# Jumpat/SegAnyGAussians

Measured on AMD Instinct MI355X. Metric: train views/sec (fwd+bwd), 1080p, 1M Gaussians, 32-D features, higher is better.
Workload: dtype f32; 1 GPU; BASELINE cfg3: 1000000 Gaussians, 1920x1080, 32-D features, fwd+bwd, 1 view/GPU/step; parallelism=view-sharded x1

## Files before the change

### seganygaussians_amd/csrc/binning.h

```cpp
#pragma once

#include <type_traits>

#include "common.h"
#include "cull.h"

namespace mirast {

__device__ __forceinline__ uint32_t wave_inclusive_scan(uint32_t v, int lane)
{
#pragma unroll
    for (int o = 1; o < 64; o <<= 1) {
        const uint32_t t = __shfl_up(v, o, 64);
        if (lane >= o) v += t;
    }
    return v;
}

template <int CTRL, int ROW_MASK, int BANK_MASK>
__device__ __forceinline__ uint32_t dpp_or_zero(uint32_t v)
{
    return (uint32_t)__builtin_amdgcn_update_dpp(0, (int)v, CTRL, ROW_MASK, BANK_MASK, false);
}
template <bool MAX = false>
// ... 17 lines not shown

struct RectWork {
    uint32_t* prefix;
    uint32_t* rx;
    uint32_t* ry;
    uint32_t* wsum;
};

template <int NT = 1024, typename F>
__device__ __forceinline__ void for_each_tile_balanced(const RectWork& rw, int tid, uint2 rmin, uint2 rmax, uint32_t count, F&& f)
{
    const int lane = tid & 63, wave = tid >> 6;
    uint32_t incl = wave_inclusive_scan(count, lane);
    if (lane == 63) rw.wsum[wave] = incl;
    __syncthreads();
    uint32_t woff = 0, total = 0;
#pragma unroll
    for (int w = 0; w < NT / 64; w++) {
        const uint32_t c = rw.wsum[w];
        woff += w < wave ? c : 0u;
        total += c;
    }
    incl += woff;
    rw.prefix[tid] = incl;
    rw.rx[tid] = rmin.x | ((rmax.x - rmin.x) << 16);
    rw.ry[tid] = rmin.y;
    __syncthreads();
    for (uint32_t k = (uint32_t)tid; k < total; k += NT) {
        int lo = 0;
#pragma unroll
        for (int step = NT / 2; step >= 1; step >>= 1)
            if (rw.prefix[lo + step - 1] <= k) lo += step;
        const uint32_t packed = rw.rx[lo];
        const uint32_t w = packed >> 16, x0 = packed & 0xFFFFu, y0 = rw.ry[lo];
        const uint32_t prev = lo == 0 ? 0u : rw.prefix[lo - 1];
        const uint32_t i = k - prev;
        const uint32_t row = (uint32_t)(((float)i + 0.5f) * __builtin_amdgcn_rcpf((float)w));
        const uint32_t col = i - row * w;
        f((uint32_t)lo, x0 + col, y0 + row);
    }
    __syncthreads();
}

constexpr int ID_BITS = 28;
constexpr uint32_t ID_MASK = (1u << ID_BITS) - 1u;
constexpr int BIN_MAX_WG = 256;
constexpr int BIN_THREADS = 1024;
constexpr int BIN_LEAN_WG = 256;
constexpr int BIN_MAX_TILES = 22 * 1024 - 64;
constexpr int BIN_MAX_TILES_TOTAL = 40 * 1024 - 128;

__host__ __device__ inline bool band_geometry(uint32_t gx, uint32_t gy, uint32_t max_head_words, uint32_t& band_h, uint32_t& nbands)
{
    band_h = (gy + 15u) / 16u;
    if (band_h < 1u) band_h = 1u;
    while (band_h > 1u && (band_h + 1u) * (gx + 2u) > max_head_words) band_h--;
    nbands = (gy + band_h - 1u) / band_h;
    return nbands <= (uint32_t)MAX_BANDS && (band_h + 1u) * (gx + 2u) <= max_head_words;
}

__device__ __forceinline__ void band_plan(const int* __restrict__ r_slots, uint32_t nbands, uint32_t nwg, uint32_t* s_plan, int lane)
{
    uint32_t cnt = 0;
    if ((uint32_t)lane < nbands)
        for (int k = 0; k < R_SLOTS; k++) cnt += (uint32_t)r_slots[k * R_SLOT_STRIDE + R_SLOT_BANDS + lane];
    uint32_t total = cnt;
#pragma unroll
    for (int o = 32; o >= 1; o >>= 1) total += (uint32_t)__shfl_xor((int)total, o, 64);
    const uint32_t avail = nwg > nbands ? nwg - nbands : 0u;
    uint32_t n = (uint32_t)lane < nbands ? 1u + (total ? (uint32_t)(((uint64_t)cnt * avail) / total) : 0u) : 0u;
    if (nwg < nbands) n = (uint32_t)lane < nwg ? 1u : 0u;
    uint32_t incl = n;
#pragma unroll
    for (int o = 1; o < 64; o <<= 1) {
        const uint32_t t = (uint32_t)__shfl_up((int)incl, o, 64);
        if (lane >= o) incl += t;
    }
    if ((uint32_t)lane < nbands) s_plan[lane] = incl - n;
    if ((uint32_t)lane == nbands) s_plan[nbands] = incl;
}

constexpr int NR_TOTAL = 0, NR_LONGEST = 1, NR_VERIFY = 2, NR_KEY_BITS = 3, NR_RUN_BOUNDS = 4;

__global__ void __launch_bounds__(1024) tile_ranges_kernel(int ntiles_all, const uint32_t* __restrict__ tile_total,
                                                           uint2* __restrict__ ranges, int* __restrict__ num_rendered,
                                                           const int* __restrict__ r_slots, int* __restrict__ host_out = nullptr,
                                                           uint32_t* __restrict__ zero_a = nullptr, uint32_t* __restrict__ zero_b = nullptr,
                                                           uint32_t* __restrict__ run_bounds = nullptr ,
                                                           uint32_t run_cap = 0, uint32_t run_fix = 0)
{
    extern __shared__ uint32_t s_val[];
    __shared__ uint32_t s_wave[16];
    __shared__ uint32_t s_wave_w[16];
    __shared__ uint32_t s_bound[9];
    const bool weighted = run_bounds != nullptr && run_cap > 0u && ntiles_all <= BIN_MAX_TILES_TOTAL;
    __shared__ uint32_t s_maxcount;
    const int tid = threadIdx.x, lane = tid & 63, wave = tid >> 6;
    if (tid < 9) s_bound[tid] = xcd_run_start((uint32_t)tid, (uint32_t)ntiles_all);
    if (tid == 0) s_maxcount = 0;
    if (wave == 15 && r_slots != nullptr) {
        uint32_t inv_min = (uint32_t)r_slots[(lane % R_SLOTS) * R_SLOT_STRIDE + 1];
        uint32_t mx = (uint32_t)r_slots[(lane % R_SLOTS) * R_SLOT_STRIDE + 2];
#pragma unroll
        for (int o = 32; o >= 1; o >>= 1) {
            inv_min = max(inv_min, (uint32_t)__shfl_xor((int)inv_min, o, 64));
            mx = max(mx, (uint32_t)__shfl_xor((int)mx, o, 64));
        }
        const uint32_t kmin = ~inv_min;
        const uint32_t diff = mx >= kmin ? (mx ^ kmin) : 0u;
        if (lane == 0) num_rendered[NR_KEY_BITS] = diff ? 32 - __builtin_clz(diff) : 0;
    }
    uint32_t carry = 0;
    for (int seg0 = 0; seg0 < ntiles_all; seg0 += BIN_MAX_TILES_TOTAL) {
        const int ntiles = min(BIN_MAX_TILES_TOTAL, ntiles_all - seg0);
        for (int i = tid; i < ntiles; i += 1024) s_val[i] = tile_total[seg0 + i];
        __syncthreads();
        const int per = (ntiles + 1023) / 1024;
        const int i0 = min(ntiles, tid * per), i1 = min(ntiles, i0 + per);
        uint32_t sum = 0, mx = 0, wsum = 0;
        for (int i = i0; i < i1; i++) {
            const uint32_t c = s_val[i];
            s_val[i] = sum;
            sum += c;
            mx = max(mx, c);
            wsum += min(c, run_cap) + run_fix;
        }
        const uint32_t incl = wave_inclusive_scan(sum, lane);
        const uint32_t incl_w = weighted ? wave_inclusive_scan(wsum, lane) : 0u;
        if (lane == 63) {
            s_wave[wave] = incl;
            s_wave_w[wave] = incl_w;
        }
#pragma unroll
        for (int o = 32; o >= 1; o >>= 1) mx = max(mx, (uint32_t)__shfl_xor((int)mx, o, 64));
        __syncthreads();
        if (lane == 0 && mx) atomicMax(&s_maxcount, mx);
        uint32_t woff = 0, total = 0;
#pragma unroll
        for (int w = 0; w < 16; w++) {
            const uint32_t c = s_wave[w];
            woff += w < wave ? c : 0u;
            total += c;
        }
        const uint32_t piece_base = carry + woff + incl - sum;
        for (int i = i0; i < i1; i++) s_val[i] += piece_base;
        if (tid == 0) s_val[ntiles] = carry + total;
        uint32_t woff_w = 0, total_w = 0;
        if (weighted) {
#pragma unroll
            for (int w = 0; w < 16; w++) {
                const uint32_t c = s_wave_w[w];
                woff_w += w < wave ? c : 0u;
                total_w += c;
            }
        }
        __syncthreads();
        if (weighted && total_w > 0u) {
            const uint64_t w_lo = 8ull * (uint64_t)(woff_w + incl_w - wsum), w_hi = 8ull * (uint64_t)(woff_w + incl_w);
#pragma unroll
            for (uint32_t k = 1; k < 8u; k++) {
                const uint64_t want = (uint64_t)k * (uint64_t)total_w;
                if (w_lo < want && want <= w_hi) {
                    uint64_t wacc = w_lo;
                    int i = i0;
                    for (; i < i1; i++) {
                        wacc += 8ull * (uint64_t)(min(s_val[i + 1] - s_val[i], run_cap) + run_fix);
                        if (wacc >= want) break;
                    }
                    s_bound[k] = (uint32_t)min(i + 1, i1);
                }
            }
        }
        for (int i = tid; i < ntiles; i += 1024) {
            const uint32_t lo = s_val[i], hi = s_val[i + 1];
            ranges[seg0 + i] = hi > lo ? make_uint2(lo, hi) : make_uint2(0u, 0u);
            if (zero_a != nullptr) {
                zero_a[seg0 + i] = 0u;
                zero_b[seg0 + i] = 0u;
            }
        }
        carry += total;
        __syncthreads();
    }
    if (run_bounds != nullptr) {
        const uint32_t n = (uint32_t)ntiles_all;
        if (tid == 0) {
            uint32_t bb[9];
#pragma unroll
            for (int k = 1; k < 8; k++) bb[k] = s_bound[k];
            const uint32_t maxrun = xcd_max_run(n);
            bb[0] = 0u;
            bb[8] = n;
#pragma unroll
            for (uint32_t k = 1; k < 8u; k++) {
                const uint32_t prev = bb[k - 1], need = (8u - k) * maxrun;
                bb[k] = min(max(bb[k], max(prev, n > need ? n - need : 0u)), min(n, prev + maxrun));
            }
#pragma unroll
            for (int k = 0; k < 9; k++) {
                run_bounds[k] = bb[k];
                if (host_out != nullptr) host_out[NR_RUN_BOUNDS + k] = (int)bb[k];
            }
        }
    }
    if (tid == 0) {
        num_rendered[NR_TOTAL] = (int)carry;
        num_rendered[NR_LONGEST] = (int)s_maxcount;
        if (host_out != nullptr) {
            host_out[NR_TOTAL] = (int)carry;
            host_out[NR_LONGEST] = (int)s_maxcount;
        }
    }
}

constexpr int MI_FP_MAX = 8;
constexpr int FP_BLOCKS = 128;
struct FingerprintArgs {
    const uint32_t* ptr[MI_FP_MAX];
    unsigned long long words[MI_FP_MAX];
};
__global__ void __launch_bounds__(256) fingerprint_kernel(FingerprintArgs a, unsigned long long* __restrict__ out)
{
    const int k = blockIdx.y;
    const uint32_t* p = a.ptr[k];
    const unsigned long long n = a.words[k];
    unsigned long long sum = 0;
    for (unsigned long long i = (unsigned long long)blockIdx.x * 256ull + threadIdx.x; i < n; i += (unsigned long long)FP_BLOCKS * 256ull) {
        uint32_t x = p[i] ^ ((uint32_t)i * 0x9E3779B1u + (uint32_t)(i >> 32));
        x ^= x >> 16;
        x *= 0x85EBCA6Bu;
        x ^= x >> 13;
        x *= 0xC2B2AE35u;
        x ^= x >> 16;
        sum += (unsigned long long)x * 0x9E3779B97F4A7C15ull + i;
    }
    __shared__ unsigned long long s_part[4];
#pragma unroll
    for (int o = 32; o >= 1; o >>= 1) sum += __shfl_xor(sum, o, 64);
    if ((threadIdx.x & 63) == 0) s_part[threadIdx.x >> 6] = sum;
    __syncthreads();
    if (threadIdx.x == 0) out[k * FP_BLOCKS + blockIdx.x] = s_part[0] + s_part[1] + s_part[2] + s_part[3];
}

__global__ void __launch_bounds__(256) reuse_image_state_kernel(uint32_t ntiles, const uint2* __restrict__ src_ranges,
                                                                const int* __restrict__ src_words, uint2* __restrict__ ranges,
                                                                int* __restrict__ words, uint32_t* __restrict__ zero_a,
                                                                uint32_t* __restrict__ zero_b)
{
    const uint32_t t = blockIdx.x * 256u + threadIdx.x;
    if (t < ntiles) {
        ranges[t] = src_ranges[t];
        zero_a[t] = 0u;
        zero_b[t] = 0u;
    }
    if (t < 16u) words[t] = src_words[t];
}

struct __attribute__((aligned(16))) BlendRec {
    float2 xy;
    uint32_t id;
    uint32_t pm;
    float4 co;
};
static_assert(sizeof(BlendRec) == 32, "BlendRec must be 32 bytes");

__device__ __forceinline__ BlendRec list_record(const uint32_t* __restrict__ lst, const BlendRec* __restrict__ index_rec, int i)
{
    const uint32_t e = lst[i];
    BlendRec r = index_rec[e & ID_MASK];
    r.id = e & ID_MASK;
    r.pm = ((uint32_t)i << 4) | (e >> ID_BITS);
    return r;
}

inline int bin_workgroups(int P)
{
    const int blocks = (P + BIN_THREADS - 1) / BIN_THREADS;
    return blocks < 1 ? 1 : (blocks > BIN_MAX_WG ? BIN_MAX_WG : blocks);
}

template <bool NOCULL = false>
__global__ void __launch_bounds__(BIN_THREADS) bin_ranks_kernel(int P, const BlendRec* __restrict__ index_rec,
                                                                const uint32_t* __restrict__ depth_key,
                                                                const uint32_t* __restrict__ partial,
                                                                const uint2* __restrict__ ranges,
                                                                uint2* __restrict__ entries, uint32_t gx, uint32_t gy,
                                                                uint32_t by0, uint32_t by1)
{
    extern __shared__ uint32_t s_dyn[];
    const int ntiles = (int)(gx * (by1 - by0));
    const int tile0 = (int)(gx * by0);
    const int ntiles_all = (int)(gx * gy);
    uint32_t* s_cnt = s_dyn;
// ... 681 lines not shown
```

### seganygaussians_amd/csrc/geometry.h

```cpp
#pragma once

#include "binning.h"
#include "common.h"

namespace mirast {

__device__ constexpr float SH_C0 = 0.28209479177387814f;
__device__ constexpr float SH_C1 = 0.4886025119029199f;
__device__ constexpr float SH_C2[5] = {1.0925484305920792f, -1.0925484305920792f, 0.31539156525252005f,
                                       -1.0925484305920792f, 0.5462742152960396f};
__device__ constexpr float SH_C3[7] = {-0.5900435899266435f, 2.890611442640554f, -0.4570457994644658f,
                                       0.3731763325901154f, -0.4570457994644658f, 1.445305721320277f,
                                       -0.5900435899266435f};

__device__ __forceinline__ void computeCov3D(const float3 scale, float mod, const float4 rot, float* cov3D)
{
    Mat3 S = {{{1.0f, 0, 0}, {0, 1.0f, 0}, {0, 0, 1.0f}}};
    S.m[0][0] = mod * scale.x;
    S.m[1][1] = mod * scale.y;
    S.m[2][2] = mod * scale.z;
    float r = rot.x, x = rot.y, y = rot.z, z = rot.w;
    Mat3 R = {{{1.f - 2.f * (y * y + z * z), 2.f * (x * y - r * z), 2.f * (x * z + r * y)},
               {2.f * (x * y + r * z), 1.f - 2.f * (x * x + z * z), 2.f * (y * z - r * x)},
               {2.f * (x * z - r * y), 2.f * (y * z + r * x), 1.f - 2.f * (x * x + y * y)}}};
// ... 5 lines not shown
    cov3D[3] = Sigma.m[1][1];
    cov3D[4] = Sigma.m[1][2];
    cov3D[5] = Sigma.m[2][2];
}

struct Cov2DCtx {
    float3 t;
    float txtz, tytz;
    Mat3 T, Vrk, W, cov;
};

__device__ __forceinline__ void cov2d_common(const float3& mean, const ViewParams& vp, const float* cov3D, Cov2DCtx& c)
{
    float3 t = transformPoint4x3(mean, vp.view);
    const float limx = 1.3f * vp.tan_fovx;
    const float limy = 1.3f * vp.tan_fovy;
    c.txtz = t.x / t.z;
    c.tytz = t.y / t.z;
    t.x = fminf(limx, fmaxf(-limx, c.txtz)) * t.z;
    t.y = fminf(limy, fmaxf(-limy, c.tytz)) * t.z;
    Mat3 J = {{{vp.focal_x / t.z, 0.0f, -(vp.focal_x * t.x) / (t.z * t.z)},
               {0.0f, vp.focal_y / t.z, -(vp.focal_y * t.y) / (t.z * t.z)},
               {0, 0, 0}}};
    c.W = {{{vp.view[0], vp.view[4], vp.view[8]}, {vp.view[1], vp.view[5], vp.view[9]}, {vp.view[2], vp.view[6], vp.view[10]}}};
    c.T = m3mul(c.W, J);
    c.Vrk = {{{cov3D[0], cov3D[1], cov3D[2]}, {cov3D[1], cov3D[3], cov3D[4]}, {cov3D[2], cov3D[4], cov3D[5]}}};
    c.cov = m3mul(m3mul(m3transpose(c.T), m3transpose(c.Vrk)), c.T);
    c.cov.m[0][0] += 0.3f;
    c.cov.m[1][1] += 0.3f;
    c.t = t;
}

__device__ __forceinline__ float3 computeColorFromSH(int idx, int deg, const float3 pos, const ViewParams& vp,
                                                     const float* sh, uint8_t* clamped)
{
    float3 dir = make_float3(pos.x - vp.campos[0], pos.y - vp.campos[1], pos.z - vp.campos[2]);
    float len = sqrtf(dir.x * dir.x + dir.y * dir.y + dir.z * dir.z);
    dir.x = dir.x / len;
    dir.y = dir.y / len;
    dir.z = dir.z / len;
    const float x = dir.x, y = dir.y, z = dir.z;
    float res[3];
#pragma unroll
    for (int c = 0; c < 3; c++) {
#define SH(k) sh[(k) * 3 + c]
        float result = SH_C0 * SH(0);
        if (deg > 0) {
            result = result - SH_C1 * y * SH(1) + SH_C1 * z * SH(2) - SH_C1 * x * SH(3);
            if (deg > 1) {
                float xx = x * x, yy = y * y, zz = z * z;
                float xy = x * y, yz = y * z, xz = x * z;
                result = result + SH_C2[0] * xy * SH(4) + SH_C2[1] * yz * SH(5) + SH_C2[2] * (2.0f * zz - xx - yy) * SH(6) +
                         SH_C2[3] * xz * SH(7) + SH_C2[4] * (xx - yy) * SH(8);
                if (deg > 2) {
                    result = result + SH_C3[0] * y * (3.0f * xx - yy) * SH(9) + SH_C3[1] * xy * z * SH(10) +
                             SH_C3[2] * y * (4.0f * zz - xx - yy) * SH(11) +
                             SH_C3[3] * z * (2.0f * zz - 3.0f * xx - 3.0f * yy) * SH(12) +
                             SH_C3[4] * x * (4.0f * zz - xx - yy) * SH(13) + SH_C3[5] * z * (xx - yy) * SH(14) +
                             SH_C3[6] * x * (xx - 3.0f * yy) * SH(15);
                }
            }
        }
#undef SH
        result += 0.5f;
        clamped[3 * idx + c] = (result < 0);
        res[c] = fmaxf(result, 0.0f);
    }
    return make_float3(res[0], res[1], res[2]);
}

__global__ void __launch_bounds__(256) preprocess_fwd_kernel(
    int P, int D, int M, const float* __restrict__ orig_points, const float* __restrict__ scales,
    const float* __restrict__ rotations, const float* __restrict__ opacities, const float* __restrict__ shs,
    uint8_t* __restrict__ clamped, const float* __restrict__ cov3D_precomp, int colors_given, ViewParams vp,
    int* __restrict__ radii, float2* __restrict__ points_xy_image, float* __restrict__ depths,
    float* __restrict__ cov3Ds, float* __restrict__ rgb, float4* __restrict__ conic_opacity,
    uint32_t* __restrict__ tiles_touched, uint32_t* __restrict__ depth_key, BlendRec* __restrict__ index_rec,
    int* __restrict__ r_slots, int prefiltered, int* __restrict__ culled_prefiltered, unsigned long long* __restrict__ band_bits,
    uint32_t band_h, uint32_t nbands, uint32_t* __restrict__ tile_total, uint32_t ntiles)
{
    const int idx = blockIdx.x * blockDim.x + threadIdx.x;
    __shared__ uint32_t s_band[MAX_BANDS];
    if (threadIdx.x < MAX_BANDS) s_band[threadIdx.x] = 0u;
    if ((uint32_t)idx < ntiles) tile_total[idx] = 0u;
    extern __shared__ float s_sh[];
    const int sh_row = 3 * M + 4;
    if (!colors_given) {
        const int rows = min((int)blockDim.x, P - (int)(blockIdx.x * blockDim.x));
        const size_t base = (size_t)blockIdx.x * blockDim.x * 3 * M;
        const int nfl = rows * 3 * M;
        if ((3 * M) % 4 == 0 && (reinterpret_cast<uintptr_t>(shs) & 15) == 0) {
            for (int i = 4 * (int)threadIdx.x; i < nfl; i += 4 * (int)blockDim.x) {
                const float4 v = *reinterpret_cast<const float4*>(shs + base + i);
                *reinterpret_cast<float4*>(&s_sh[(i / (3 * M)) * sh_row + i % (3 * M)]) = v;
            }
        } else {
            for (int i = (int)threadIdx.x; i < nfl; i += (int)blockDim.x) s_sh[(i / (3 * M)) * sh_row + i % (3 * M)] = shs[base + i];
        }
        __syncthreads();
    }
    int my_radii = 0;
    uint32_t my_tiles = 0;
    uint32_t my_key = 0xFFFFFFFFu;
    uint2 rect_min = make_uint2(0, 0), rect_max = make_uint2(0, 0);
    if (idx < P) do {
        const float3 p_orig = make_float3(orig_points[3 * idx], orig_points[3 * idx + 1], orig_points[3 * idx + 2]);
        const float3 p_view = transformPoint4x3(p_orig, vp.view);
        if (p_view.z <= 0.2f) {
            if (prefiltered) atomicAdd(culled_prefiltered, 1);
            break;
        }
        const float4 p_hom = transformPoint4x4(p_orig, vp.proj);
        const float p_w = 1.0f / (p_hom.w + 0.0000001f);
        const float3 p_proj = make_float3(p_hom.x * p_w, p_hom.y * p_w, p_hom.z * p_w);

        float cov3D[6];
        if (cov3D_precomp != nullptr) {
#pragma unroll
            for (int i = 0; i < 6; i++) cov3D[i] = cov3D_precomp[(size_t)idx * 6 + i];
        } else {
            const float3 s = make_float3(scales[3 * idx], scales[3 * idx + 1], scales[3 * idx + 2]);
            const float4 q = reinterpret_cast<const float4*>(rotations)[idx];
            computeCov3D(s, vp.scale_modifier, q, cov3D);
#pragma unroll
            for (int i = 0; i < 6; i++) cov3Ds[(size_t)idx * 6 + i] = cov3D[i];
        }
        Cov2DCtx c;
        cov2d_common(p_orig, vp, cov3D, c);
        const float3 cov = make_float3(c.cov.m[0][0], c.cov.m[0][1], c.cov.m[1][1]);
        const float det = (cov.x * cov.z - cov.y * cov.y);
        if (det == 0.0f) break;
        const float det_inv = 1.f / det;
        const float3 conic = make_float3(cov.z * det_inv, -cov.y * det_inv, cov.x * det_inv);
        const float mid = 0.5f * (cov.x + cov.z);
        const float lambda1 = mid + sqrtf(fmaxf(0.1f, mid * mid - det));
        const float lambda2 = mid - sqrtf(fmaxf(0.1f, mid * mid - det));
        const float my_radius = ceilf(3.f * sqrtf(fmaxf(lambda1, lambda2)));
        const float2 point_image = make_float2(ndc2Pix(p_proj.x, vp.W), ndc2Pix(p_proj.y, vp.H));
        uint2 rmin, rmax;
        getRect(point_image.x, point_image.y, f2i(my_radius), rmin, rmax, vp.grid_x, vp.grid_y);
        if ((rmax.x - rmin.x) * (rmax.y - rmin.y) == 0) break;

        if (!colors_given) {
            const float3 col = computeColorFromSH(idx, D, p_orig, vp, s_sh + threadIdx.x * sh_row, clamped);
            rgb[idx * 3 + 0] = col.x;
            rgb[idx * 3 + 1] = col.y;
            rgb[idx * 3 + 2] = col.z;
        }
        depths[idx] = p_view.z;
        my_radii = f2i(my_radius);
        points_xy_image[idx] = point_image;
        conic_opacity[idx] = make_float4(conic.x, conic.y, conic.z, opacities[idx]);
        my_tiles = (rmax.y - rmin.y) * (rmax.x - rmin.x);
        if (my_radii > 0) {
            getRect(point_image.x, point_image.y, my_radii, rect_min, rect_max, vp.grid_x, vp.grid_y);
            my_key = __float_as_uint(p_view.z);
            BlendRec rec;
            rec.xy = point_image;
            rec.id = my_key;
            rec.pm = (uint32_t)my_radii;
            rec.co = make_float4(conic.x, conic.y, conic.z, opacities[idx]);
            index_rec[idx] = rec;
        }
    } while (0);
    uint32_t my_bands = 0u;
    if (my_radii > 0 && rect_max.y > rect_min.y && rect_max.x > rect_min.x) {
        const uint32_t b0 = rect_min.y / band_h, b1 = (rect_max.y - 1u) / band_h;
// ... 318 lines not shown
```

### seganygaussians_amd/csrc/mi_rast.hip

```cpp
#include "../../include/mi_rast.h"
#include "../../include/mi_knn_smooth.h"
#include "../../include/mi_knn.h"
#include "../../include/mi_contrastive.h"
#include "../../include/mi_mask_scales.h"
#include "../../include/mi_segment.h"
#include "../../include/mi_photometric.h"

#include <hip/hip_runtime.h>

#include <algorithm>
#include <atomic>
#include <cstdio>
#include <cstdlib>
#include <cstring>
#include <mutex>
#include <string>
#include <vector>

#include "binning.h"
#include "knn_smooth.h"
#include "knn.h"
#include "blend_bwd.h"
#include "blend_bwd_wave.h"
#include "blend_bwd_feat.h"
// ... 208 lines not shown
    mi_rast_image_layout(W, H, off);
    ImgPtrs m;
    m.final_T = (float*)(base + off[MI_IMG_FINAL_T]);
    m.n_contrib = (uint32_t*)(base + off[MI_IMG_N_CONTRIB]);
    m.ranges = (uint2*)(base + off[MI_IMG_RANGES]);
    m.tile_consumed = (uint32_t*)(base + off[MI_IMG_TILE_CONSUMED]);
    m.tile_count = (uint32_t*)(base + off[MI_IMG_TILE_COUNT]);
    m.tile_cursor = (uint32_t*)(base + off[MI_IMG_TILE_CURSOR]);
    m.num_rendered = (int*)(base + off[MI_IMG_NUM_RENDERED]);
    m.tile_nsurv = (uint32_t*)(base + off[MI_IMG_TILE_NSURV]);
    m.run_bounds = reinterpret_cast<uint32_t*>(m.num_rendered + R_SLOTS * R_SLOT_STRIDE + NR_RUN_BOUNDS);
    m.longest_run = 0;
    return m;
}
BinPtrs bin_from(char* base, int R)
{
    size_t off[MI_BIN_NFIELDS];
    mi_rast_binning_layout(R, off);
    BinPtrs b;
    b.entries = (uint2*)(base + off[MI_BIN_ENTRIES]);
    b.scratch = (uint2*)(base + off[MI_BIN_SCRATCH]);
    b.blend_list = (uint32_t*)(base + off[MI_BIN_BLEND_LIST]);
    return b;
}

std::atomic<bool> g_attr_set[MAX_DEVICES];
std::mutex g_attr_mutex;

constexpr int MAX_CHANNELS = 256;
constexpr int MAX_CHANNEL_BLOCKS = MAX_CHANNELS / 16;
inline size_t bwd_pack_bytes(int P)
{
    return (size_t)(P > 0 ? P : 1) * 8 * sizeof(float) + MAX_CHANNEL_BLOCKS * 8 * XCD_QUEUE_STRIDE * sizeof(uint32_t);
}
bool channels_supported(int c) { return c >= 1 && c <= MAX_CHANNELS; }
int channel_block(int rem) { return rem >= 64 ? 64 : (rem >= 32 ? 32 : 16); }

constexpr int RUN_MODEL_CAP = 768;
constexpr int RUN_MODEL_FIX = 128;
inline uint32_t longest_of(const int* bounds, uint32_t ntiles)
{
    uint32_t longest = 0;
    for (int x = 0; x < 8; x++) {
        const uint32_t a = (uint32_t)bounds[x], b = (uint32_t)bounds[x + 1];
        longest = std::max(longest, b >= a ? b - a : 0u);
    }
    return std::min(std::max(longest, (ntiles + 7u) >> 3), xcd_max_run(ntiles));
}

int geometry_and_binning(mi_rast_resize_fn geometry_buffer, void* geometry_user, mi_rast_resize_fn binning_buffer,
                         void* binning_user, mi_rast_resize_fn image_buffer, void* image_user, int P, int D, int M,
                         int W, int H, const float* means3D, const float* shs, int colors_given,
                         const float* opacities, const float* scales, const float* rotations,
                         const float* cov3D_precomp, const ViewParams& vp, int prefiltered, int* radii, int debug,
                         int flags, hipStream_t stream, GeomPtrs& geom, ImgPtrs& img, BinPtrs& bin, int* num_rendered)
{
    const int dev = current_device();
    if (dev < 0) return fail(MI_RAST_ERR_HIP, "hipGetDevice failed (or device ordinal >= 64)");
    HostSync& g_host_sync = g_host_sync_tl[dev];
    size_t goff[MI_GEOM_NFIELDS], ioff[MI_IMG_NFIELDS];
    const size_t geom_size = mi_rast_geometry_layout(P, goff);
    char* geom_base = geometry_buffer(geom_size, geometry_user);
    if (!geom_base) return fail(MI_RAST_ERR_ALLOC, "geometry buffer callback returned NULL");
    geom = geom_from(geom_base, P);
    const size_t img_size = mi_rast_image_layout(W, H, ioff);
    char* img_base = image_buffer(img_size, image_user);
    if (!img_base) return fail(MI_RAST_ERR_ALLOC, "image buffer callback returned NULL");
    img = img_from(img_base, W, H);

    int* cull_counter = geom.cull_counter;
    if (prefiltered) HIP_TRY(hipMemsetAsync(cull_counter, 0, sizeof(int), stream));
    const int ntiles = (int)(vp.grid_x * vp.grid_y);
    if (P >= (1 << ID_BITS)) return fail(MI_RAST_ERR_INVALID, "more than 2^28 Gaussians");
    if (vp.grid_x > 1023u || vp.grid_y > 2047u)
        return fail(MI_RAST_ERR_INVALID, "image too large: more than 1023 tiles across or 2047 tiles down");
    const uint32_t band_rows = std::min<uint32_t>(vp.grid_y, std::max<uint32_t>(1u, (uint32_t)BIN_MAX_TILES / (vp.grid_x + 2u) - 1u));
    const uint32_t nbands = (vp.grid_y + band_rows - 1) / band_rows;
    uint32_t lean_band_h = 1, lean_nbands = 1;
    if (!band_geometry(vp.grid_x, vp.grid_y, SPAN_MAX_HEAD_WORDS, lean_band_h, lean_nbands))
        return fail(MI_RAST_ERR_INVALID, "image too large for the banded binning passes (more than 24 bands of tile rows at this width)");
    {
        StageTimer t(stream, MI_STAGE_PREPROCESS);
        HIP_TRY(hipMemsetAsync(img.num_rendered, 0, R_SLOTS * R_SLOT_STRIDE * sizeof(int), stream));
        if (P < ntiles) HIP_TRY(hipMemsetAsync(img.tile_cursor, 0, (size_t)ntiles * sizeof(uint32_t), stream));
        const size_t sh_lds = colors_given ? 0 : (size_t)256 * (3 * (size_t)M + 4) * sizeof(float);
        if (sh_lds > 64 * 1024) return fail(MI_RAST_ERR_INVALID, "too many SH coefficients per Gaussian (at most 16: degree 3)");
        hipLaunchKernelGGL(preprocess_fwd_kernel, dim3((P + 255) / 256), dim3(256), sh_lds, stream, P, D, M, means3D, scales,
                           rotations, opacities, shs, geom.clamped, cov3D_precomp, colors_given, vp, radii,
                           geom.means2D, geom.depths, geom.cov3D, geom.rgb, geom.conic_opacity, geom.tiles_touched,
                           geom.depth_key, geom.index_rec, img.num_rendered, prefiltered, cull_counter, geom.band_bits, lean_band_h, lean_nbands,
                           img.tile_cursor, (uint32_t)ntiles);
    }
    STAGE_CHECK("preprocess");
    if (prefiltered) {
        int culled = 0;
        HIP_TRY(hipMemcpyAsync(&culled, cull_counter, sizeof(int), hipMemcpyDeviceToHost, stream));
        HIP_TRY(hipStreamSynchronize(stream));
        if (culled)
            return fail(MI_RAST_ERR_INVALID, "Point is filtered although prefiltered is set. This shouldn't happen!");
    }
    if (!g_attr_set[dev].load(std::memory_order_acquire)) {
        std::lock_guard<std::mutex> lock(g_attr_mutex);
        if (!g_attr_set[dev].load(std::memory_order_relaxed)) {
            const int max_lds = (int)((BIN_MAX_TILES + 11 * 1024 + 16) * sizeof(uint32_t));
            HIP_TRY(hipFuncSetAttribute((const void*)bin_ranks_kernel<false>, hipFuncAttributeMaxDynamicSharedMemorySize, max_lds));
            HIP_TRY(hipFuncSetAttribute((const void*)bin_ranks_kernel<true>, hipFuncAttributeMaxDynamicSharedMemorySize, max_lds));
            HIP_TRY(hipFuncSetAttribute((const void*)bin_count_kernel, hipFuncAttributeMaxDynamicSharedMemorySize, max_lds));
            HIP_TRY(hipFuncSetAttribute((const void*)bin_spans_kernel<false>, hipFuncAttributeMaxDynamicSharedMemorySize, 160 * 1024 - 256));
            HIP_TRY(hipFuncSetAttribute((const void*)bin_spans_kernel<true>, hipFuncAttributeMaxDynamicSharedMemorySize, 160 * 1024 - 256));
            HIP_TRY(hipFuncSetAttribute((const void*)tile_ranges_kernel, hipFuncAttributeMaxDynamicSharedMemorySize,
                                        (BIN_MAX_TILES_TOTAL + 1) * (int)sizeof(uint32_t)));
            g_attr_set[dev].store(true, std::memory_order_release);
        }
    }
    if (!g_host_sync.init()) return fail(MI_RAST_ERR_HIP, "cannot allocate pinned host buffer / event");
    const bool nocull = (flags & MI_RAST_NO_CULL) != 0;
    const bool full = debug != 0 || nocull || (flags & MI_RAST_FULL_LISTS) != 0;
    const int nwg = full ? bin_workgroups(P) : std::min(BIN_LEAN_WG, (int)lean_nbands + (P + 1023) / 1024);
    const size_t band_tiles = (size_t)band_rows * vp.grid_x;
    const size_t bin_lds = ((size_t)((band_tiles + 3) & ~(size_t)3) + 3 * 1024 + 16) * sizeof(uint32_t);
    {
        StageTimer t(stream, MI_STAGE_TILE_SCAN);
        const size_t cnt_lds = (size_t)(band_rows + 1) * count_grid_stride(vp.grid_x) * sizeof(int);
        for (uint32_t b = 0; full && b < nbands; b++) {
            const uint32_t by0 = b * band_rows, by1 = std::min(vp.grid_y, by0 + band_rows);
            if (full)
                hipLaunchKernelGGL(bin_count_kernel, dim3(nwg), dim3(BIN_THREADS), cnt_lds, stream, P, geom.index_rec, geom.depth_key,
                                   img.tile_count, vp.grid_x, vp.grid_y, by0, by1, (const int*)img.num_rendered,
                                   b == 0 ? g_host_sync.pinned_dev : (int*)nullptr);
        }
        if (!full)
            hipLaunchKernelGGL(bin_spans_kernel<false>, dim3(nwg), dim3(1024), span_lds_bytes((size_t)lean_band_h * count_grid_stride(vp.grid_x)),
                               stream, P, geom.index_rec, geom.depth_key, geom.band_bits, img.tile_count, img.tile_cursor, (const uint2*)nullptr, (uint2*)nullptr,
                               vp.grid_x, vp.grid_y, lean_band_h, lean_nbands, (const int*)img.num_rendered, g_host_sync.pinned_dev);
        HIP_TRY(hipEventRecord(g_host_sync.ev, stream));
        if (full)
            hipLaunchKernelGGL(scan_partials_kernel, dim3((ntiles + 63) / 64), dim3(1024), 0, stream, ntiles, nwg,
                               img.tile_count, img.tile_cursor);
        const uint32_t run_cap = !(flags & MI_RAST_EQUAL_RUNS) ? (uint32_t)RUN_MODEL_CAP : 0u;
        const uint32_t run_fix = (uint32_t)RUN_MODEL_FIX;
        hipLaunchKernelGGL(tile_ranges_kernel, dim3(1), dim3(1024),
                           ((size_t)std::min(ntiles, BIN_MAX_TILES_TOTAL) + 1) * sizeof(uint32_t), stream, ntiles, img.tile_cursor,
                           img.ranges, img.num_rendered + R_SLOTS * R_SLOT_STRIDE, (const int*)img.num_rendered,
                           g_host_sync.pinned_dev + R_SLOTS * R_SLOT_STRIDE, img.tile_consumed, img.tile_nsurv, img.run_bounds, run_cap, run_fix);
    }
    STAGE_CHECK("tile scan");
    HIP_TRY(hipEventRecord(g_host_sync.ev2, stream));
    HIP_TRY(hipEventSynchronize(g_host_sync.ev));
    long long Rsum = 0;
    for (int k = 0; k < R_SLOTS; k++) Rsum += g_host_sync.pinned[k * R_SLOT_STRIDE];
    if (Rsum > 0x7fffffffll) return fail(MI_RAST_ERR_INVALID, "more than 2^31 tile overlaps");
    const int R = (int)Rsum;
    *num_rendered = R;

    size_t boff[MI_BIN_NFIELDS];
    const size_t bin_size = mi_rast_binning_layout(R, boff);
    char* bin_base = binning_buffer(bin_size, binning_user);
    if (!bin_base) return fail(MI_RAST_ERR_ALLOC, "binning buffer callback returned NULL");
    bin = bin_from(bin_base, R);
    const bool verify = !full && (flags & MI_RAST_VERIFY_LISTS) != 0;
    if (R > 0) {
        if (verify) HIP_TRY(hipMemsetAsync(bin.entries, 0, (size_t)R * sizeof(uint2), stream));
        {
            StageTimer t(stream, MI_STAGE_EMIT);
            const size_t emit_lds = bin_lds + 8 * 1024 * sizeof(uint32_t);
            for (uint32_t b = 0; full && b < nbands; b++) {
                const uint32_t by0 = b * band_rows, by1 = std::min(vp.grid_y, by0 + band_rows);
                if (nocull)
                    hipLaunchKernelGGL(bin_ranks_kernel<true>, dim3(nwg), dim3(BIN_THREADS), emit_lds, stream, P, geom.index_rec, geom.depth_key,
                                       img.tile_count, img.ranges, bin.entries, vp.grid_x, vp.grid_y, by0, by1);
                else if (full)
                    hipLaunchKernelGGL(bin_ranks_kernel<false>, dim3(nwg), dim3(BIN_THREADS), emit_lds, stream, P, geom.index_rec, geom.depth_key,
                                       img.tile_count, img.ranges, bin.entries, vp.grid_x, vp.grid_y, by0, by1);
            }
            if (!full)
                hipLaunchKernelGGL(bin_spans_kernel<true>, dim3(nwg), dim3(1024), span_lds_bytes((size_t)lean_band_h * vp.grid_x), stream, P,
                                   geom.index_rec, geom.depth_key, geom.band_bits, img.tile_count, img.tile_cursor, img.ranges, bin.entries, vp.grid_x, vp.grid_y,
                                   lean_band_h, lean_nbands, (const int*)img.num_rendered, (int*)nullptr);
        }
        STAGE_CHECK("emit entries");
        if (verify) {
            uint32_t* ctr = reinterpret_cast<uint32_t*>(img.num_rendered + R_SLOTS * R_SLOT_STRIDE + NR_VERIFY);
            HIP_TRY(hipMemsetAsync(ctr, 0, sizeof(uint32_t), stream));
            hipLaunchKernelGGL(verify_entries_kernel, dim3(ntiles), dim3(256), 0, stream, (uint32_t)ntiles, img.ranges, bin.entries, ctr);
            uint32_t unwritten = 0;
            HIP_TRY(hipMemcpyAsync(&unwritten, ctr, sizeof(uint32_t), hipMemcpyDeviceToHost, stream));
            HIP_TRY(hipStreamSynchronize(stream));
            if (unwritten)
                return fail(MI_RAST_ERR_HIP, "internal error: " + std::to_string(unwritten) + " list slots were counted but not emitted "
                                             "(count / emit passes of bin_spans_kernel disagree)");
        }
        const int* key_bits = img.num_rendered + R_SLOTS * R_SLOT_STRIDE + NR_KEY_BITS;
        {
            StageTimer t(stream, MI_STAGE_TILE_SORT);
#define LAUNCH_TILE_SORT(LO, CAP, FB, NT)                                                                                 \
    hipLaunchKernelGGL((tile_sort_kernel<LO, CAP, FB, NT>), dim3(ntiles), dim3(NT), 0, stream, (uint32_t)ntiles, img.ranges,  \
                       bin.entries, bin.scratch, key_bits, bin.blend_list)
            hipLaunchKernelGGL(tile_sort_wave_kernel<0>, dim3((ntiles + 3) / 4), dim3(256), 0, stream, (uint32_t)ntiles, img.ranges,
                               (const uint2*)bin.entries, bin.blend_list);
            HIP_TRY(hipEventSynchronize(g_host_sync.ev2));
            img.longest_run = longest_of(g_host_sync.pinned + R_SLOTS * R_SLOT_STRIDE + NR_RUN_BOUNDS, (uint32_t)ntiles);
            g_last_longest_run[dev] = (int)img.longest_run;
            if (full ? g_host_sync.pinned[R_SLOTS * R_SLOT_STRIDE + NR_TOTAL] != R : g_host_sync.pinned[R_SLOTS * R_SLOT_STRIDE + NR_TOTAL] > R)
                return fail(MI_RAST_ERR_HIP, "internal error: tile counts do not add up to num_rendered");
            const int max_tile_count = g_host_sync.pinned[R_SLOTS * R_SLOT_STRIDE + NR_LONGEST];
            if (max_tile_count > 1024)
                hipLaunchKernelGGL(tile_sort_wave_kernel<1>, dim3((ntiles + 3) / 4), dim3(256), 0, stream, (uint32_t)ntiles, img.ranges,
                                   (const uint2*)bin.entries, bin.blend_list);
            if (max_tile_count > 2048)
                hipLaunchKernelGGL(tile_sort_wave_kernel<2>, dim3((ntiles + 3) / 4), dim3(256), 0, stream, (uint32_t)ntiles, img.ranges,
                                   (const uint2*)bin.entries, bin.blend_list);
            if (max_tile_count > TILE_SORT_WAVE_MAX) LAUNCH_TILE_SORT(TILE_SORT_WAVE_MAX, 6144, false, 1024);
            if (max_tile_count > 6144) LAUNCH_TILE_SORT(6144, 8192, true, 1024);
#undef LAUNCH_TILE_SORT
        }
        STAGE_CHECK("tile sort");
    } else {
        HIP_TRY(hipEventSynchronize(g_host_sync.ev2));
        img.longest_run = longest_of(g_host_sync.pinned + R_SLOTS * R_SLOT_STRIDE + NR_RUN_BOUNDS, (uint32_t)ntiles);
        g_last_longest_run[dev] = (int)img.longest_run;
    }
    return MI_RAST_OK;
}

template <int C, int EXTRA>
// ... 1128 lines not shown
```

Baseline: 928.6 views/s.

## Parallelize tile range scan across workgroups and fold tile_total zeroing into preprocess

The single 1024-thread workgroup that scanned tile counts, wrote ranges and computed run bounds is split. Block 0 now computes only totals, the longest count and the weighted run bounds. The other blocks each redo a prefix sum over the tiles before their slice and write their own ranges. The preprocess kernel now zeroes tile_total with a grid-stride loop, which removes a separate memset. This spreads a serial single-block pass across many CUs, at the cost of redundant prefix reads of tile_total in each block.

```diff
diff --git a/seganygaussians_amd/csrc/binning.h b/seganygaussians_amd/csrc/binning.h
--- a/seganygaussians_amd/csrc/binning.h
+++ b/seganygaussians_amd/csrc/binning.h
@@ -123,23 +123,73 @@
 
 constexpr int NR_TOTAL = 0, NR_LONGEST = 1, NR_VERIFY = 2, NR_KEY_BITS = 3, NR_RUN_BOUNDS = 4;
 
-__global__ void __launch_bounds__(1024) tile_ranges_kernel(int ntiles_all, const uint32_t* __restrict__ tile_total,
-                                                           uint2* __restrict__ ranges, int* __restrict__ num_rendered,
-                                                           const int* __restrict__ r_slots, int* __restrict__ host_out = nullptr,
-                                                           uint32_t* __restrict__ zero_a = nullptr, uint32_t* __restrict__ zero_b = nullptr,
-                                                           uint32_t* __restrict__ run_bounds = nullptr ,
-                                                           uint32_t run_cap = 0, uint32_t run_fix = 0)
-{
+constexpr int RANGE_THREADS = 256;
+constexpr int RANGE_MAX_WG = 64;
+inline int range_workgroups(int ntiles)
+{
+    const int n = (ntiles + RANGE_THREADS - 1) / RANGE_THREADS;
+    return n < 1 ? 1 : (n > RANGE_MAX_WG ? RANGE_MAX_WG : n);
+}
+inline size_t range_lds_bytes(int ntiles) { return ntiles <= BIN_MAX_TILES_TOTAL ? (size_t)ntiles * sizeof(uint32_t) : 0; }
+
+__global__ void __launch_bounds__(RANGE_THREADS) tile_ranges_kernel(int ntiles_all, const uint32_t* __restrict__ tile_total,
+                                                                    uint2* __restrict__ ranges, int* __restrict__ num_rendered,
+                                                                    const int* __restrict__ r_slots, int* __restrict__ host_out = nullptr,
+                                                                    uint32_t* __restrict__ zero_a = nullptr, uint32_t* __restrict__ zero_b = nullptr,
+                                                                    uint32_t* __restrict__ run_bounds = nullptr ,
+                                                                    uint32_t run_cap = 0, uint32_t run_fix = 0)
+{
+    constexpr int NT = RANGE_THREADS, NW = RANGE_THREADS / 64;
     extern __shared__ uint32_t s_val[];
-    __shared__ uint32_t s_wave[16];
-    __shared__ uint32_t s_wave_w[16];
+    __shared__ uint32_t s_front[NW];
+    __shared__ uint32_t s_wave[2][NW];
+    __shared__ uint32_t s_sum[NW], s_max[NW], s_wave_w[NW];
     __shared__ uint32_t s_bound[9];
+    const int tid = threadIdx.x, lane = tid & 63, wave = tid >> 6;
+    if (blockIdx.x != 0) {
+        const int nrb = (int)gridDim.x - 1, b = (int)blockIdx.x - 1;
+        const int per_wg = (ntiles_all + nrb - 1) / nrb;
+        const int start = min(ntiles_all, b * per_wg), end = min(ntiles_all, start + per_wg);
+        uint32_t front = 0;
+        for (int i = tid; i < start; i += NT) front += tile_total[i];
+#pragma unroll
+        for (int o = 32; o >= 1; o >>= 1) front += (uint32_t)__shfl_xor((int)front, o, 64);
+        if (lane == 0) s_front[wave] = front;
+        uint32_t carry = 0;
+        int pass = 0;
+        for (int r0 = start; r0 < end; r0 += NT, pass++) {
+            const int i = r0 + tid;
+            const uint32_t c = i < end ? tile_total[i] : 0u;
+            const uint32_t incl = wave_inclusive_scan_dpp(c);
+            uint32_t* sw = s_wave[pass & 1];
+            if (lane == 63) sw[wave] = incl;
+            __syncthreads();
+            if (pass == 0) {
+#pragma unroll
+                for (int w = 0; w < NW; w++) carry += s_front[w];
+            }
+            uint32_t woff = 0, total = 0;
+#pragma unroll
+            for (int w = 0; w < NW; w++) {
+                const uint32_t t = sw[w];
+                woff += w < wave ? t : 0u;
+                total += t;
+            }
+            if (i < end) {
+                const uint32_t lo = carry + woff + incl - c, hi = lo + c;
+                ranges[i] = hi > lo ? make_uint2(lo, hi) : make_uint2(0u, 0u);
+                if (zero_a != nullptr) {
+                    zero_a[i] = 0u;
+                    zero_b[i] = 0u;
+                }
+            }
+            carry += total;
+        }
+        return;
+    }
     const bool weighted = run_bounds != nullptr && run_cap > 0u && ntiles_all <= BIN_MAX_TILES_TOTAL;
-    __shared__ uint32_t s_maxcount;
-    const int tid = threadIdx.x, lane = tid & 63, wave = tid >> 6;
     if (tid < 9) s_bound[tid] = xcd_run_start((uint32_t)tid, (uint32_t)ntiles_all);
-    if (tid == 0) s_maxcount = 0;
-    if (wave == 15 && r_slots != nullptr) {
+    if (wave == NW - 1 && r_slots != nullptr) {
         uint32_t inv_min = (uint32_t)r_slots[(lane % R_SLOTS) * R_SLOT_STRIDE + 1];
         uint32_t mx = (uint32_t)r_slots[(lane % R_SLOTS) * R_SLOT_STRIDE + 2];
 #pragma unroll
@@ -151,81 +201,67 @@
         const uint32_t diff = mx >= kmin ? (mx ^ kmin) : 0u;
         if (lane == 0) num_rendered[NR_KEY_BITS] = diff ? 32 - __builtin_clz(diff) : 0;
     }
-    uint32_t carry = 0;
-    for (int seg0 = 0; seg0 < ntiles_all; seg0 += BIN_MAX_TILES_TOTAL) {
-        const int ntiles = min(BIN_MAX_TILES_TOTAL, ntiles_all - seg0);
-        for (int i = tid; i < ntiles; i += 1024) s_val[i] = tile_total[seg0 + i];
+    uint32_t sum = 0, mx = 0, wsum = 0;
+    int i0 = 0, i1 = 0;
+    if (weighted) {
+        for (int i = tid; i < ntiles_all; i += NT) s_val[i] = tile_total[i];
         __syncthreads();
-        const int per = (ntiles + 1023) / 1024;
-        const int i0 = min(ntiles, tid * per), i1 = min(ntiles, i0 + per);
-        uint32_t sum = 0, mx = 0, wsum = 0;
+        const int per = ((ntiles_all + NT - 1) / NT) | 1;
+        i0 = min(ntiles_all, tid * per);
+        i1 = min(ntiles_all, i0 + per);
         for (int i = i0; i < i1; i++) {
             const uint32_t c = s_val[i];
-            s_val[i] = sum;
             sum += c;
             mx = max(mx, c);
             wsum += min(c, run_cap) + run_fix;
         }
-        const uint32_t incl = wave_inclusive_scan(sum, lane);
-        const uint32_t incl_w = weighted ? wave_inclusive_scan(wsum, lane) : 0u;
-        if (lane == 63) {
-            s_wave[wave] = incl;
-            s_wave_w[wave] = incl_w;
-        }
-#pragma unroll
-        for (int o = 32; o >= 1; o >>= 1) mx = max(mx, (uint32_t)__shfl_xor((int)mx, o, 64));
-        __syncthreads();
-        if (lane == 0 && mx) atomicMax(&s_maxcount, mx);
-        uint32_t woff = 0, total = 0;
-#pragma unroll
-        for (int w = 0; w < 16; w++) {
-            const uint32_t c = s_wave[w];
-            woff += w < wave ? c : 0u;
-            total += c;
-        }
-        const uint32_t piece_base = carry + woff + incl - sum;
-        for (int i = i0; i < i1; i++) s_val[i] += piece_base;
-        if (tid == 0) s_val[ntiles] = carry + total;
-        uint32_t woff_w = 0, total_w = 0;
-        if (weighted) {
-#pragma unroll
-            for (int w = 0; w < 16; w++) {
-                const uint32_t c = s_wave_w[w];
-                woff_w += w < wave ? c : 0u;
-                total_w += c;
-            }
-        }
-        __syncthreads();
-        if (weighted && total_w > 0u) {
-            const uint64_t w_lo = 8ull * (uint64_t)(woff_w + incl_w - wsum), w_hi = 8ull * (uint64_t)(woff_w + incl_w);
-#pragma unroll
-            for (uint32_t k = 1; k < 8u; k++) {
-                const uint64_t want = (uint64_t)k * (uint64_t)total_w;
-                if (w_lo < want && want <= w_hi) {
-                    uint64_t wacc = w_lo;
-                    int i = i0;
-                    for (; i < i1; i++) {
-                        wacc += 8ull * (uint64_t)(min(s_val[i + 1] - s_val[i], run_cap) + run_fix);
-                        if (wacc >= want) break;
-                    }
-                    s_bound[k] = (uint32_t)min(i + 1, i1);
+    } else {
+        for (int i = tid; i < ntiles_all; i += NT) {
+            const uint32_t c = tile_total[i];
+            sum += c;
+            mx = max(mx, c);
+        }
+    }
+    const uint32_t incl_w = weighted ? wave_inclusive_scan_dpp(wsum) : 0u;
+#pragma unroll
+    for (int o = 32; o >= 1; o >>= 1) {
+        sum += (uint32_t)__shfl_xor((int)sum, o, 64);
+        mx = max(mx, (uint32_t)__shfl_xor((int)mx, o, 64));
+    }
+    if (lane == 63) {
+        s_sum[wave] = sum;
+        s_max[wave] = mx;
+        s_wave_w[wave] = incl_w;
+    }
+    __syncthreads();
+    uint32_t total = 0, longest = 0, woff_w = 0, total_w = 0;
+#pragma unroll
+    for (int w = 0; w < NW; w++) {
+        total += s_sum[w];
+        longest = max(longest, s_max[w]);
+        const uint32_t t = s_wave_w[w];
+        woff_w += w < wave ? t : 0u;
+        total_w += t;
+    }
+    if (weighted && total_w > 0u) {
+        const uint64_t w_lo = 8ull * (uint64_t)(woff_w + incl_w - wsum), w_hi = 8ull * (uint64_t)(woff_w + incl_w);
+        if (w_lo < 7ull * (uint64_t)total_w && (uint64_t)total_w <= w_hi) {
+            uint64_t wacc = w_lo;
+            for (int i = i0; i < i1; i++) {
+                const uint64_t prev = wacc;
+                wacc += 8ull * (uint64_t)(min(s_val[i], run_cap) + run_fix);
+#pragma unroll
+                for (uint32_t k = 1; k < 8u; k++) {
+                    const uint64_t want = (uint64_t)k * (uint64_t)total_w;
+                    if (prev < want && want <= wacc) s_bound[k] = (uint32_t)(i + 1);
                 }
             }
         }
-        for (int i = tid; i < ntiles; i += 1024) {
-            const uint32_t lo = s_val[i], hi = s_val[i + 1];
-            ranges[seg0 + i] = hi > lo ? make_uint2(lo, hi) : make_uint2(0u, 0u);
-            if (zero_a != nullptr) {
-                zero_a[seg0 + i] = 0u;
-                zero_b[seg0 + i] = 0u;
-            }
-        }
-        carry += total;
-        __syncthreads();
-    }
-    if (run_bounds != nullptr) {
-        const uint32_t n = (uint32_t)ntiles_all;
-        if (tid == 0) {
+    }
+    __syncthreads();
+    if (tid == 0) {
+        if (run_bounds != nullptr) {
+            const uint32_t n = (uint32_t)ntiles_all;
             uint32_t bb[9];
 #pragma unroll
             for (int k = 1; k < 8; k++) bb[k] = s_bound[k];
@@ -243,13 +279,11 @@
                 if (host_out != nullptr) host_out[NR_RUN_BOUNDS + k] = (int)bb[k];
             }
         }
-    }
-    if (tid == 0) {
-        num_rendered[NR_TOTAL] = (int)carry;
-        num_rendered[NR_LONGEST] = (int)s_maxcount;
+        num_rendered[NR_TOTAL] = (int)total;
+        num_rendered[NR_LONGEST] = (int)longest;
         if (host_out != nullptr) {
-            host_out[NR_TOTAL] = (int)carry;
-            host_out[NR_LONGEST] = (int)s_maxcount;
+            host_out[NR_TOTAL] = (int)total;
+            host_out[NR_LONGEST] = (int)longest;
         }
     }
 }
diff --git a/seganygaussians_amd/csrc/geometry.h b/seganygaussians_amd/csrc/geometry.h
--- a/seganygaussians_amd/csrc/geometry.h
+++ b/seganygaussians_amd/csrc/geometry.h
@@ -111,7 +111,7 @@
     const int idx = blockIdx.x * blockDim.x + threadIdx.x;
     __shared__ uint32_t s_band[MAX_BANDS];
     if (threadIdx.x < MAX_BANDS) s_band[threadIdx.x] = 0u;
-    if ((uint32_t)idx < ntiles) tile_total[idx] = 0u;
+    for (uint32_t t = (uint32_t)idx; t < ntiles; t += gridDim.x * blockDim.x) tile_total[t] = 0u;
     extern __shared__ float s_sh[];
     const int sh_row = 3 * M + 4;
     if (!colors_given) {
diff --git a/seganygaussians_amd/csrc/mi_rast.hip b/seganygaussians_amd/csrc/mi_rast.hip
--- a/seganygaussians_amd/csrc/mi_rast.hip
+++ b/seganygaussians_amd/csrc/mi_rast.hip
@@ -314,7 +314,6 @@
     {
         StageTimer t(stream, MI_STAGE_PREPROCESS);
         HIP_TRY(hipMemsetAsync(img.num_rendered, 0, R_SLOTS * R_SLOT_STRIDE * sizeof(int), stream));
-        if (P < ntiles) HIP_TRY(hipMemsetAsync(img.tile_cursor, 0, (size_t)ntiles * sizeof(uint32_t), stream));
         const size_t sh_lds = colors_given ? 0 : (size_t)256 * (3 * (size_t)M + 4) * sizeof(float);
         if (sh_lds > 64 * 1024) return fail(MI_RAST_ERR_INVALID, "too many SH coefficients per Gaussian (at most 16: degree 3)");
         hipLaunchKernelGGL(preprocess_fwd_kernel, dim3((P + 255) / 256), dim3(256), sh_lds, stream, P, D, M, means3D, scales,
@@ -341,7 +340,7 @@
             HIP_TRY(hipFuncSetAttribute((const void*)bin_spans_kernel<false>, hipFuncAttributeMaxDynamicSharedMemorySize, 160 * 1024 - 256));
             HIP_TRY(hipFuncSetAttribute((const void*)bin_spans_kernel<true>, hipFuncAttributeMaxDynamicSharedMemorySize, 160 * 1024 - 256));
             HIP_TRY(hipFuncSetAttribute((const void*)tile_ranges_kernel, hipFuncAttributeMaxDynamicSharedMemorySize,
-                                        (BIN_MAX_TILES_TOTAL + 1) * (int)sizeof(uint32_t)));
+                                        (int)range_lds_bytes(BIN_MAX_TILES_TOTAL)));
             g_attr_set[dev].store(true, std::memory_order_release);
         }
     }
@@ -371,8 +370,7 @@
                                img.tile_count, img.tile_cursor);
         const uint32_t run_cap = !(flags & MI_RAST_EQUAL_RUNS) ? (uint32_t)RUN_MODEL_CAP : 0u;
         const uint32_t run_fix = (uint32_t)RUN_MODEL_FIX;
-        hipLaunchKernelGGL(tile_ranges_kernel, dim3(1), dim3(1024),
-                           ((size_t)std::min(ntiles, BIN_MAX_TILES_TOTAL) + 1) * sizeof(uint32_t), stream, ntiles, img.tile_cursor,
+        hipLaunchKernelGGL(tile_ranges_kernel, dim3(1 + range_workgroups(ntiles)), dim3(RANGE_THREADS), range_lds_bytes(ntiles), stream, ntiles, img.tile_cursor,
                            img.ranges, img.num_rendered + R_SLOTS * R_SLOT_STRIDE, (const int*)img.num_rendered,
                            g_host_sync.pinned_dev + R_SLOTS * R_SLOT_STRIDE, img.tile_consumed, img.tile_nsurv, img.run_bounds, run_cap, run_fix);
     }
```

Result: no change. 928.1 views/s (-0.0%).
